# thiagopbueno/tf-mpc

Hardware: AMD Instinct MI355X
Metric: iLQR iterations/sec (batch x horizon) at n=16,m=8,T=50 (higher is better)
Workload: dtype f32

## Files before the change

### tf-mpc_amd/csrc/lqr_mfma16x8.hip

```cpp
#include <hip/hip_runtime.h>

#include <cstdlib>
#include <cstring>
#include <type_traits>

#include "lqr_kernels.h"
#include "options.h"
#include "mfma_bf16x3.h"
#include "wave_ldlt8.h"
#include "wave_ops.h"

namespace tfmpc {

namespace {

constexpr int N = 16, M = 8, D = 24;
using f32x4 = bf3::f32x4;

__device__ __forceinline__ f32x4 mfma(float a, float b, f32x4 c)
{
    return __builtin_amdgcn_mfma_f32_16x16x4f32(a, b, c, 0, 0, 0);
}

__device__ __forceinline__ float readlane(float v, int lane)
{
    return __builtin_bit_cast(float, __builtin_amdgcn_readlane(__builtin_bit_cast(int, v), lane));
}

using namespace bf3;

constexpr int kMs = 0;
constexpr int kKs = 256;
constexpr int kZs = 512;
constexpr int kZld = 26;
constexpr int kVtLd = 20;
#ifndef TFMPC_LQR_TC
#define TFMPC_LQR_TC 52
#endif
constexpr int kTC = TFMPC_LQR_TC;
constexpr int kLdsFloats = kZs + (kTC + 1) * kZld + 6;
#ifndef TFMPC_LQR_RING
#define TFMPC_LQR_RING 4
#endif
constexpr int kRing = TFMPC_LQR_RING;
static_assert(kTC % kRing == 0, "a chunk must hold whole turns of the gain ring");

template <int CTRL>
__device__ __forceinline__ float dpp(float v)
{
    return __builtin_bit_cast(float, __builtin_amdgcn_update_dpp(0, __builtin_bit_cast(int, v), CTRL, 0xF, 0xF, false));
}
constexpr int kDppXor1 = 0xB1;
constexpr int kDppXor2 = 0x4E;
constexpr int kDppHalfMirror = 0x141;

#define TFMPC_GLOBAL __attribute__((address_space(1)))
using gbytes = TFMPC_GLOBAL char *;
__device__ __forceinline__ gbytes uniform_base(const float *p)
{
    gbytes g = (gbytes)p;
    asm("" : "+s"(g));
    return g;
}
__device__ __forceinline__ unsigned here(unsigned &off)
{
    asm volatile("" : "+v"(off));
    return off;
}
template <class V>
__device__ __forceinline__ V gload(gbytes base, unsigned &off) { return *reinterpret_cast<const TFMPC_GLOBAL V *>(base + here(off)); }
template <class V>
__device__ __forceinline__ void gstore(gbytes base, unsigned &off, V v) { *reinterpret_cast<TFMPC_GLOBAL V *>(base + here(off)) = v; }
__device__ __forceinline__ int pinned(int v)
{
    asm("" : "+v"(v));
    return v;
}
typedef float f32x4_lds __attribute__((ext_vector_type(4), aligned(8)));
typedef float f32x4_any __attribute__((ext_vector_type(4), aligned(4)));

#ifdef TFMPC_LQR_EU
#define TFMPC_LQR_WAVES(EU_) TFMPC_LQR_EU
#else
#define TFMPC_LQR_WAVES(EU_) (EU_)
#endif
#define TFMPC_LQR_OCCUPANCY __attribute__((amdgpu_waves_per_eu(TFMPC_LQR_WAVES(EU), TFMPC_LQR_WAVES(EU))))
template <bool BACKWARD, bool FORWARD, bool VALUE, bool EXACT, bool BF3, bool OUT16 = false, int EU = 4>
__global__ __launch_bounds__(kWave) TFMPC_LQR_OCCUPANCY void lqr_mfma16x8_kernel(LqrArgs a)
{
    __shared__ __attribute__((aligned(16))) float lds[kLdsFloats];
    const int b = blockIdx.x;
    const int lane = threadIdx.x;
    const int i = lane & 15, q = lane >> 4;
    const int T = a.T;
    const int n = EXACT ? N : a.n, m = EXACT ? M : a.m, d = n + m;
    auto Fxx = [&](const float *Fg, int row, int xi) { return (row < n && xi < n) ? Fg[row * d + xi] : 0.0f; };
    auto Fxu = [&](const float *Fg, int row, int ui) { return (row < n && ui < m) ? Fg[row * d + n + ui] : 0.0f; };
    auto zmap = [&](int zi) { return zi < N ? (zi < n ? zi : -1) : (zi - N < m ? n + zi - N : -1); };
    auto Czz = [&](const float *Cg, int zr, int zc) {
        const int r = zmap(zr), c_ = zmap(zc);
        return (r >= 0 && c_ >= 0) ? Cg[r * d + c_] : 0.0f;
    };
    auto cz = [&](const float *cg, int zr) { const int r = zmap(zr); return r >= 0 ? cg[r] : 0.0f; };
    const float *Fg = a.F + (size_t)b * a.sF;
    const float *fg = a.f + (size_t)b * a.sf;
    const float *Cg = a.C + (size_t)b * a.sC;
    const float *cg = a.c + (size_t)b * a.sc;
    float *Kg = a.K + (size_t)b * a.sK;
    float *kg = a.k + (size_t)b * a.sk;
    int status = 0;

    if (BACKWARD) {
        float Fb0[4], Fb1[4];
        f32x4 Cd00, Cd11;
        f32x4 Cd01t;
        f32x4 vterm;
#pragma unroll
        for (int r = 0; r < 4; ++r) {
            const int k = 4 * q + r;
            const int ku = N + k;
            if (EXACT) {
                Fb0[r] = Fg[k * D + i];
                Fb1[r] = (i < M) ? Fg[k * D + N + i] : ((i == M) ? fg[k] : 0.0f);
                Cd00[r] = Cg[k * D + i];
                Cd01t[r] = (k < M) ? Cg[(N + k) * D + i] : ((k == M) ? cg[i] : 0.0f);
                vterm[r] = (i == M) ? cg[k] : 0.0f;
                Cd11[r] = (ku < D) ? ((i < M) ? Cg[ku * D + N + i] : ((i == M) ? cg[ku] : 0.0f)) : 0.0f;
            } else {
                Fb0[r] = Fxx(Fg, k, i);
                Fb1[r] = (i < M) ? Fxu(Fg, k, i) : ((i == M && k < n) ? fg[k] : 0.0f);
                Cd00[r] = Czz(Cg, k, i);
                Cd01t[r] = (k < M) ? Czz(Cg, N + k, i) : ((k == M) ? cz(cg, i) : 0.0f);
                vterm[r] = (i == M) ? cz(cg, k) : 0.0f;
                float c11 = 0.0f;
                if (ku < D) {
                    if (i < M) c11 = (k >= m && i == k) ? 1.0f : Czz(Cg, ku, N + i);
                    else if (i == M) c11 = cz(cg, ku);
                }
                Cd11[r] = c11;
            }
        }
        ConstFrag Fc0{}, Fc1{};
        if (BF3) {
            Fc0 = const_frag(f32x4{Fb0[0], Fb0[1], Fb0[2], Fb0[3]});
            Fc1 = const_frag(f32x4{Fb1[0], Fb1[1], Fb1[2], Fb1[3]});
        }
        f32x4 Vd = Cd00, vd = vterm;
        float cst = 0.0f;
        int min_pivot_bits = 0x3f800000;
        constexpr int kZero = kMs + 25 * 8;
        if (lane < kKs - kZero) lds[kZero + lane] = 0.0f;
        constexpr int kQx = kMs + 28 * 8;
        const int t01_src = (i == M) ? kQx + 4 * q : kZero;
        const int g1_src = (i == M) ? kKs + (N + M) * 8 + q : kZero + q;
        const int g0_src = pinned(kKs + i * 8 + q);
        const int vt_dst = pinned(kZs + 4 * q * kVtLd + i);
        unsigned offK = 8u * lane, offk = 4u * lane;
        __syncthreads();

        auto sweep_step = [&](const int t, auto LAST) __attribute__((always_inline)) {
            f32x4 W0 = {0.f, 0.f, 0.f, 0.f}, W1 = vd;
            if (BF3) {
                const VarFrag Vf = var_frag_block(Vd);
                W0 = mm_var_const(Vf, Fc0, W0);
                W1 = mm_var_const(Vf, Fc1, W1);
            } else {
#pragma unroll
                for (int r = 0; r < 4; ++r) {
                    W0 = mfma(Vd[r], Fb0[r], W0);
                    W1 = mfma(Vd[r], Fb1[r], W1);
                }
            }
            float fw = 0.0f, fv = 0.0f;
            if (VALUE) {
                float pw = 0.0f, pv = 0.0f;
#pragma unroll
                for (int r = 0; r < 4; ++r) {
                    pw = fmaf(Fb1[r], W1[r], pw);
                    pv = fmaf(Fb1[r], vd[r], pv);
                }
                fw = wave_sum(i == M ? pw : 0.0f);
                fv = wave_sum(i == M ? pv : 0.0f);
            }
            f32x4 T00 = Cd00, T01t = Cd01t, T11 = Cd11;
            if (BF3) {
                const VarFrag W0f = var_frag_block(W0), W1f = var_frag_block(W1);
                T00 = mm_const_var(Fc0, W0f, T00);
                T01t = mm_var_const(W1f, Fc0, T01t);
                T11 = mm_const_var(Fc1, W1f, T11);
            } else {
#pragma unroll
                for (int r = 0; r < 4; ++r) {
                    T00 = mfma(Fb0[r], W0[r], T00);
                    T01t = mfma(W1[r], Fb0[r], T01t);
                    T11 = mfma(Fb1[r], W1[r], T11);
                }
            }
            if (q < 2) {
                *reinterpret_cast<f32x4 *>(&lds[kMs + i * 8 + 4 * q]) = T01t;
                if (i <= M) *reinterpret_cast<f32x4 *>(&lds[kMs + (N + i) * 8 + 4 * q]) = T11;
            } else if (q == 2) {
                lds[kQx + i] = T01t[0];
            }
            lds_sync();
            f32x2 M2[4];
            {
                const int c = lane & 31;
                const f32x4 lo = *reinterpret_cast<const f32x4 *>(&lds[kMs + c * 8]);
                const f32x4 hi = *reinterpret_cast<const f32x4 *>(&lds[kMs + c * 8 + 4]);
                M2[0] = f32x2{lo[0], lo[1]}; M2[1] = f32x2{lo[2], lo[3]};
                M2[2] = f32x2{hi[0], hi[1]}; M2[3] = f32x2{hi[2], hi[3]};
            }
            float quk = 0.0f;
            float qu_saved[8];
            if (VALUE) {
#pragma unroll
                for (int p = 0; p < 8; ++p) qu_saved[p] = readlane(M2[p >> 1][p & 1], 24);
            }
            float Mr[8];
            ldlt8_solve_neg(M2, Mr, min_pivot_bits);
            if (VALUE) {
#pragma unroll
                for (int p = 0; p < 8; ++p) quk = fmaf(readlane(Mr[p], 24), qu_saved[p], quk);
            }
            if (lane < 32) {
                f32x4 lo, hi;
#pragma unroll
                for (int r = 0; r < 4; ++r) { lo[r] = Mr[r]; hi[r] = Mr[4 + r]; }
                *reinterpret_cast<f32x4 *>(&lds[kKs + lane * 8]) = lo;
                *reinterpret_cast<f32x4 *>(&lds[kKs + lane * 8 + 4]) = hi;
            }
            lds_sync();
            if constexpr (!decltype(LAST)::value) {
                f32x4 vacc = *reinterpret_cast<const f32x4 *>(&lds[t01_src]);
#pragma unroll
                for (int s2 = 0; s2 < 2; ++s2) {
                    const float ax = lds[kMs + i * 8 + 4 * s2 + q];
                    const float g0 = lds[g0_src + 4 * s2];
                    const float g1 = lds[g1_src + 4 * s2];
                    T00 = mfma(ax, g0, T00);
                    vacc = mfma(ax, g1, vacc);
                }
                {
                    const float *vt = &lds[kZs];
#pragma unroll
                    for (int r = 0; r < 4; ++r) lds[vt_dst + r * kVtLd] = T00[r];
                    lds_sync();
                    const f32x4 Tt = *reinterpret_cast<const f32x4 *>(&vt[i * kVtLd + 4 * q]);
#pragma unroll
                    for (int r = 0; r < 4; ++r) Vd[r] = 0.5f * (T00[r] + Tt[r]);
                }
                vd = vacc;
            }
            {
                const int ka = lane >> 3, jc = lane & 7;
                float2 kv;
                kv.x = lds[kKs + (2 * jc) * 8 + ka];
                kv.y = lds[kKs + (2 * jc + 1) * 8 + ka];
                if (EXACT) {
                    gstore(uniform_base(Kg + (size_t)t * (M * N)), offK, f32x2{kv.x, kv.y});
                    if (lane < M) gstore(uniform_base(kg + (size_t)t * M), offk, lds[kKs + 24 * 8 + lane]);
                } else {
                    if (ka < m && 2 * jc < n) Kg[(size_t)t * m * n + ka * n + 2 * jc] = kv.x;
                    if (ka < m && 2 * jc + 1 < n) Kg[(size_t)t * m * n + ka * n + 2 * jc + 1] = kv.y;
                    if (lane < m) kg[(size_t)t * m + lane] = lds[kKs + 24 * 8 + lane];
                }
                if (OUT16 && a.K16) {
                    uint16_t *Ko = a.K16 + ((size_t)b * T + t) * (m * n);
                    if (ka < m && 2 * jc < n) Ko[ka * n + 2 * jc] = lqr_to_bf16(kv.x);
                    if (ka < m && 2 * jc + 1 < n) Ko[ka * n + 2 * jc + 1] = lqr_to_bf16(kv.y);
                }
                if (OUT16 && a.k16 && lane < m) a.k16[((size_t)b * T + t) * m + lane] = lqr_to_bf16(lds[kKs + 24 * 8 + lane]);
            }
            if (VALUE) {
                cst += 0.5f * quk + 0.5f * (fw + fv);
                if (a.V) {
                    float *Vo = a.V + ((size_t)b * T + t) * (n * n);
#pragma unroll
                    for (int r = 0; r < 4; ++r)
                        if (EXACT || (4 * q + r < n && i < n)) Vo[(4 * q + r) * n + i] = Vd[r];
                }
                if (a.v && i == M) {
                    float *vo = a.v + ((size_t)b * T + t) * n;
#pragma unroll
                    for (int r = 0; r < 4; ++r)
                        if (EXACT || 4 * q + r < n) vo[4 * q + r] = vd[r];
                }
                if (a.cst && lane == 0) a.cst[(size_t)b * T + t] = cst;
                if (OUT16 && a.V16) {
                    uint16_t *Vo = a.V16 + ((size_t)b * T + t) * (n * n);
#pragma unroll
                    for (int r = 0; r < 4; ++r)
                        if (EXACT || (4 * q + r < n && i < n)) Vo[(4 * q + r) * n + i] = lqr_to_bf16(Vd[r]);
                }
                if (OUT16 && a.v16 && i == M) {
                    uint16_t *vo = a.v16 + ((size_t)b * T + t) * n;
#pragma unroll
                    for (int r = 0; r < 4; ++r)
                        if (EXACT || 4 * q + r < n) vo[4 * q + r] = lqr_to_bf16(vd[r]);
                }
                if (OUT16 && a.cst16 && lane == 0) a.cst16[(size_t)b * T + t] = lqr_to_bf16(cst);
            }
            lds_sync();
        };
        constexpr int kPeeled = VALUE ? 0 : 1;
        for (int t = T - 1; t >= kPeeled; --t) sweep_step(t, std::false_type{});
        if (kPeeled && T > 0) sweep_step(0, std::true_type{});
        if (min_pivot_bits <= 0) status |= (min_pivot_bits == 0) ? TFMPC_ST_SINGULAR : TFMPC_ST_NOT_PD;
        if (VALUE && !(cst == cst)) status |= TFMPC_ST_NAN;
    }

    if (FORWARD) {
        const int fi = lane >> 2, fc = lane & 3;
        const int ka = lane >> 3, jc = lane & 7;
        float Fr[6];
        if (EXACT) {
            const float2 *p = reinterpret_cast<const float2 *>(Fg + fi * D + 6 * fc);
#pragma unroll
            for (int j = 0; j < 3; ++j) { const float2 v = p[j]; Fr[2 * j] = v.x; Fr[2 * j + 1] = v.y; }
        } else {
#pragma unroll
            for (int j = 0; j < 6; ++j) {
                const int zc = 6 * fc + j;
                Fr[j] = zc < N ? Fxx(Fg, fi, zc) : Fxu(Fg, fi, zc - N);
            }
        }
        const float f_part = (fc == 0 && (EXACT || fi < n)) ? fg[fi] : 0.0f;
        float Ca0[6], Ca1[6];
        f32x4 cq0, cq1;
#pragma unroll
        for (int s2 = 0; s2 < 6; ++s2) {
            if (EXACT) {
                Ca0[s2] = Cg[i * D + 4 * s2 + q];
                Ca1[s2] = (i < M) ? Cg[(N + i) * D + 4 * s2 + q] : 0.0f;
            } else {
                Ca0[s2] = Czz(Cg, i, 4 * s2 + q);
                Ca1[s2] = (i < M) ? Czz(Cg, N + i, 4 * s2 + q) : 0.0f;
            }
        }
#pragma unroll
        for (int r = 0; r < 4; ++r) {
            cq0[r] = EXACT ? cg[4 * q + r] : cz(cg, 4 * q + r);
            cq1[r] = (q < 2) ? (EXACT ? cg[N + 4 * q + r] : cz(cg, N + 4 * q + r)) : 0.0f;
        }
        float *xs = a.states + (size_t)b * (T + 1) * n;
        float *us = a.actions + (size_t)b * T * m;
        float *cs = a.costs + (size_t)b * (T + 1);
        float *zs = &lds[kZs];
        __syncthreads();
        if (lane < N) {
            const float x = (EXACT || lane < n) ? a.x0[(size_t)b * n + lane] : 0.0f;
            zs[lane] = x;
            if (EXACT || lane < n) xs[lane] = x;
        }
        unsigned offK = 8u * lane, offk = 4u * ka;
        auto load_gain = [&](int t, float2 &Kv, float &kv) {
            if (EXACT) {
                const f32x2 K2 = gload<f32x2>(uniform_base(Kg + (size_t)t * (M * N)), offK);
                Kv = float2{K2[0], K2[1]};
                kv = gload<float>(uniform_base(kg + (size_t)t * M), offk);
            } else {
                const bool row = ka < m;
                Kv.x = (row && 2 * jc < n) ? Kg[(size_t)t * m * n + ka * n + 2 * jc] : 0.0f;
                Kv.y = (row && 2 * jc + 1 < n) ? Kg[(size_t)t * m * n + ka * n + 2 * jc + 1] : 0.0f;
                kv = row ? kg[(size_t)t * m + ka] : 0.0f;
            }
        };
        float2 KR[kRing];
        float kR[kRing];
#pragma unroll
        for (int d = 0; d < kRing; ++d) {
            KR[d] = float2{0.f, 0.f};
            kR[d] = 0.0f;
            if (T > 0) load_gain(d < T ? d : T - 1, KR[d], kR[d]);
        }
        __syncthreads();

        auto chunk_costs = [&](int rows, float *out) {
            for (int nt = 0; nt * 16 < rows; ++nt) {
                const int row = (16 * nt + i < rows) ? 16 * nt + i : rows - 1;
                const float *zrow = zs + row * kZld;
                f32x4 D0 = {0.f, 0.f, 0.f, 0.f}, D1 = {0.f, 0.f, 0.f, 0.f};
#pragma unroll
                for (int s2 = 0; s2 < 6; ++s2) {
                    const float bz = zrow[4 * s2 + q];
                    D0 = mfma(Ca0[s2], bz, D0);
                    D1 = mfma(Ca1[s2], bz, D1);
                }
                float part = 0.0f;
#pragma unroll
                for (int r = 0; r < 4; ++r) {
                    part = fmaf(zrow[4 * q + r], fmaf(0.5f, D0[r], cq0[r]), part);
                    if (q < 2) part = fmaf(zrow[N + 4 * q + r], fmaf(0.5f, D1[r], cq1[r]), part);
                }
                part += __shfl_xor(part, 16, kWave);
                part += __shfl_xor(part, 32, kWave);
                if (q == 0 && 16 * nt + i < rows) out[16 * nt + i] = part;
            }
        };

        auto rollout_step = [&](const int tt, const int t, float2 &KRd, float &kRd, auto REFILL) __attribute__((always_inline)) {
            float *zt = zs + tt * kZld;
            const float2 Kc = KRd;
            const float kc = kRd;
            const float2 xv = *reinterpret_cast<const float2 *>(&zt[2 * jc]);
            float u = fmaf(Kc.x, xv.x, Kc.y * xv.y);
            u += dpp<kDppXor1>(u);
            u += dpp<kDppXor2>(u);
            u += dpp<kDppHalfMirror>(u);
            u += kc;
            if constexpr (decltype(REFILL)::value) load_gain(t + kRing < T ? t + kRing : T - 1, KRd, kRd);
            zt[N + ka] = u;
            lds_sync();
            float xn = f_part;
            const float2 *zp = reinterpret_cast<const float2 *>(&zt[6 * fc]);
#pragma unroll
            for (int j = 0; j < 3; ++j) {
                const float2 z2 = zp[j];
                xn = fmaf(Fr[2 * j], z2.x, xn);
                xn = fmaf(Fr[2 * j + 1], z2.y, xn);
            }
            xn += dpp<kDppXor1>(xn);
            xn += dpp<kDppXor2>(xn);
            zt[kZld + fi] = xn;
            lds_sync();
        };

        const int xrow = lane >> 2, urow = lane >> 1;
        const float *xsrc = zs + (1 + xrow) * kZld + 4 * (lane & 3);
        const float *usrc = zs + urow * kZld + N + 4 * (lane & 1);
        unsigned off16 = 16u * lane;

        for (int t0 = 0; t0 < T; t0 += kTC) {
            const int tc = (T - t0 < kTC) ? (T - t0) : kTC;
            int tb = 0;
            for (; tb + kRing <= tc; tb += kRing) {
#pragma unroll
                for (int d = 0; d < kRing; ++d) rollout_step(tb + d, t0 + tb + d, KR[d], kR[d], std::true_type{});
            }
#pragma unroll
            for (int d = 0; d < kRing - 1; ++d)
                if (tb + d < tc) rollout_step(tb + d, t0 + tb + d, KR[d], kR[d], std::false_type{});
            chunk_costs(tc, cs + t0);
            if (EXACT) {
                const gbytes xdst = uniform_base(xs + (size_t)(t0 + 1) * N), udst = uniform_base(us + (size_t)t0 * M);
#pragma unroll
                for (int r0 = 0; r0 < kTC; r0 += kWave / 4) {
                    if (r0 >= tc) break;
                    if (r0 + xrow < tc)
                        gstore<f32x4_any>(xdst + r0 * (N * 4), off16, *reinterpret_cast<const f32x4_lds *>(xsrc + r0 * kZld));
                }
#pragma unroll
                for (int r0 = 0; r0 < kTC; r0 += kWave / 2) {
                    if (r0 >= tc) break;
                    if (r0 + urow < tc)
                        gstore<f32x4_any>(udst + r0 * (M * 4), off16, *reinterpret_cast<const f32x4_lds *>(usrc + r0 * kZld));
                }
            } else {
                for (int idx = lane; idx < tc * n; idx += kWave)
                    xs[(size_t)(t0 + 1) * n + idx] = zs[(1 + idx / n) * kZld + idx % n];
                for (int idx = lane; idx < tc * m; idx += kWave)
                    us[(size_t)t0 * m + idx] = zs[(idx / m) * kZld + N + idx % m];
            }
            lds_sync();
            if (lane < N) zs[lane] = zs[tc * kZld + lane];
            lds_sync();
        }
        if (lane < M) zs[N + lane] = 0.0f;
        lds_sync();
        chunk_costs(1, cs + T);
        lds_sync();
        if (lane == 0) {
            const float fcost = cs[T];
            if (!(fcost == fcost)) status |= TFMPC_ST_NAN;
        }
    }

    if (a.status && lane == 0) a.status[b] = status;
}

bool use_bf16x3()
{
    return !option_is(kOptLqrMfma, "f32");
}

int pick_eu()
{
    const int forced = option_int(kOptLqrWaves, 0);
    return forced == 4 ? 4 : 5;
}

template <bool BW, bool FW, bool VAL, bool O16, int EU>
int launch_eu(const LqrArgs &a, hipStream_t stream)
{
    const bool exact = a.n == N && a.m == M;
    const bool bf3 = BW && use_bf16x3();
    const dim3 grid(a.B), block(kWave);
    if (exact && bf3) hipLaunchKernelGGL((lqr_mfma16x8_kernel<BW, FW, VAL, true, true, O16, EU>), grid, block, 0, stream, a);
    else if (exact) hipLaunchKernelGGL((lqr_mfma16x8_kernel<BW, FW, VAL, true, false, O16, EU>), grid, block, 0, stream, a);
    else if (bf3) hipLaunchKernelGGL((lqr_mfma16x8_kernel<BW, FW, VAL, false, true, O16, EU>), grid, block, 0, stream, a);
    else hipLaunchKernelGGL((lqr_mfma16x8_kernel<BW, FW, VAL, false, false, O16, EU>), grid, block, 0, stream, a);
    return hipGetLastError() == hipSuccess ? TFMPC_OK : TFMPC_ERR_LAUNCH;
}

template <bool BW, bool FW, bool VAL, bool O16 = false>
int launch(const LqrArgs &a, hipStream_t stream)
{
    if constexpr (!VAL) {
        if (pick_eu() == 5) return launch_eu<BW, FW, VAL, O16, 5>(a, stream);
    }
    return launch_eu<BW, FW, VAL, O16, 4>(a, stream);
}

}

bool lqr_mfma_supported(int n, int m) { return n >= 1 && m >= 1 && n <= N && m <= M && n + m > 6; }

int lqr_mfma_launch(const LqrArgs &a, bool backward, bool forward, hipStream_t stream)
{
    if (a.K16 || a.k16 || a.V16 || a.v16 || a.cst16) {
        if (backward && forward) return launch<true, true, true, true>(a, stream);
        if (backward) return launch<true, false, true, true>(a, stream);
    }
    const bool value = a.V || a.v || a.cst;
    if (backward && forward) return value ? launch<true, true, true>(a, stream) : launch<true, true, false>(a, stream);
    if (backward) return value ? launch<true, false, true>(a, stream) : launch<true, false, false>(a, stream);
    return launch<false, true, false>(a, stream);
}

}
```

Baseline: 39.95 million.

## Pair two batch elements per workgroup and alternate LDLT solve between waves

Launches two waves per workgroup, each handling its own batch element in the backward sweep without value outputs. The 8x8 LDLT elimination is replaced by a paired variant in which one wave, alternating by time step, solves both elements' systems using DPP row broadcasts, one element per 32-lane half. Block barriers synchronize the two waves around the solve, and pivot minima are merged at the end. This targets the poorly utilized serial solve on the critical path, at the cost of workgroup-wide barriers, doubled LDS per block and a dead wave when B is odd.

```diff
diff --git a/tf-mpc_amd/csrc/lqr_mfma16x8.hip b/tf-mpc_amd/csrc/lqr_mfma16x8.hip
--- a/tf-mpc_amd/csrc/lqr_mfma16x8.hip
+++ b/tf-mpc_amd/csrc/lqr_mfma16x8.hip
@@ -8,6 +8,7 @@
 #include "options.h"
 #include "mfma_bf16x3.h"
 #include "wave_ldlt8.h"
+#include "wave_ldlt8_pair.h"
 #include "wave_ops.h"
 
 namespace tfmpc {
@@ -85,12 +86,23 @@
 #define TFMPC_LQR_WAVES(EU_) (EU_)
 #endif
 #define TFMPC_LQR_OCCUPANCY __attribute__((amdgpu_waves_per_eu(TFMPC_LQR_WAVES(EU), TFMPC_LQR_WAVES(EU))))
-template <bool BACKWARD, bool FORWARD, bool VALUE, bool EXACT, bool BF3, bool OUT16 = false, int EU = 4>
-__global__ __launch_bounds__(kWave) TFMPC_LQR_OCCUPANCY void lqr_mfma16x8_kernel(LqrArgs a)
-{
-    __shared__ __attribute__((aligned(16))) float lds[kLdsFloats];
-    const int b = blockIdx.x;
-    const int lane = threadIdx.x;
+__device__ __forceinline__ void block_lds_sync()
+{
+    __builtin_amdgcn_fence(__ATOMIC_RELEASE, "workgroup", "local");
+    __builtin_amdgcn_s_barrier();
+    __builtin_amdgcn_fence(__ATOMIC_ACQUIRE, "workgroup", "local");
+}
+template <bool BACKWARD, bool FORWARD, bool VALUE, bool EXACT, bool BF3, bool OUT16 = false, int EU = 4, bool PAIR = false>
+__global__ __launch_bounds__(PAIR ? 2 * kWave : kWave) TFMPC_LQR_OCCUPANCY void lqr_mfma16x8_kernel(LqrArgs a)
+{
+    static_assert(!PAIR || (BACKWARD && !VALUE && !OUT16), "the paired elimination serves the sweeps without value outputs");
+    __shared__ __attribute__((aligned(16))) float lds_all[(PAIR ? 2 : 1) * kLdsFloats];
+    const int wave = PAIR ? __builtin_amdgcn_readfirstlane(threadIdx.x >> 6) : 0;
+    float *const lds = lds_all + wave * kLdsFloats;
+    const int b_own = PAIR ? 2 * (int)blockIdx.x + wave : (int)blockIdx.x;
+    const bool live = !PAIR || b_own < a.B;
+    const int b = live ? b_own : a.B - 1;
+    const int lane = PAIR ? (int)(threadIdx.x & (kWave - 1)) : (int)threadIdx.x;
     const int i = lane & 15, q = lane >> 4;
     const int T = a.T;
     const int n = EXACT ? N : a.n, m = EXACT ? M : a.m, d = n + m;
@@ -148,6 +160,11 @@
         f32x4 Vd = Cd00, vd = vterm;
         float cst = 0.0f;
         int min_pivot_bits = 0x3f800000;
+        int min_pivot_rows = 0x3f800000;
+        const int pj = lane & 15, prow = (lane >> 4) & 1;
+        const int pcol = pj >= 8 ? pj - 8 + 8 * prow : ((prow && pj == 0) ? N + M : N + pj);
+        const int pair_src = PAIR ? 4 * pinned(((lane >> 5) * kLdsFloats + kMs + pcol * 8) / 4) : 0;
+        const int pair_d0 = (lane >> 5) * kLdsFloats + kMs + N * 8;
         constexpr int kZero = kMs + 25 * 8;
         if (lane < kKs - kZero) lds[kZero + lane] = 0.0f;
         constexpr int kQx = kMs + 28 * 8;
@@ -202,35 +219,55 @@
             } else if (q == 2) {
                 lds[kQx + i] = T01t[0];
             }
-            lds_sync();
-            f32x2 M2[4];
-            {
-                const int c = lane & 31;
-                const f32x4 lo = *reinterpret_cast<const f32x4 *>(&lds[kMs + c * 8]);
-                const f32x4 hi = *reinterpret_cast<const f32x4 *>(&lds[kMs + c * 8 + 4]);
-                M2[0] = f32x2{lo[0], lo[1]}; M2[1] = f32x2{lo[2], lo[3]};
-                M2[2] = f32x2{hi[0], hi[1]}; M2[3] = f32x2{hi[2], hi[3]};
-            }
             float quk = 0.0f;
-            float qu_saved[8];
-            if (VALUE) {
-#pragma unroll
-                for (int p = 0; p < 8; ++p) qu_saved[p] = readlane(M2[p >> 1][p & 1], 24);
-            }
-            float Mr[8];
-            ldlt8_solve_neg(M2, Mr, min_pivot_bits);
-            if (VALUE) {
-#pragma unroll
-                for (int p = 0; p < 8; ++p) quk = fmaf(readlane(Mr[p], 24), qu_saved[p], quk);
-            }
-            if (lane < 32) {
-                f32x4 lo, hi;
-#pragma unroll
-                for (int r = 0; r < 4; ++r) { lo[r] = Mr[r]; hi[r] = Mr[4 + r]; }
-                *reinterpret_cast<f32x4 *>(&lds[kKs + lane * 8]) = lo;
-                *reinterpret_cast<f32x4 *>(&lds[kKs + lane * 8 + 4]) = hi;
-            }
-            lds_sync();
+            if constexpr (PAIR) {
+                block_lds_sync();
+                if (wave == (t & 1)) {
+                    f32x2 P2[4];
+                    const f32x4 lo = *reinterpret_cast<const f32x4 *>(&lds_all[pair_src]);
+                    const f32x4 hi = *reinterpret_cast<const f32x4 *>(&lds_all[pair_src + 4]);
+                    const float d0 = lds_all[pair_d0];
+                    P2[0] = f32x2{lo[0], lo[1]}; P2[1] = f32x2{lo[2], lo[3]};
+                    P2[2] = f32x2{hi[0], hi[1]}; P2[3] = f32x2{hi[2], hi[3]};
+                    float Pr[8];
+                    ldlt8_pair_solve_neg(P2, Pr, d0, min_pivot_rows);
+                    f32x4 klo, khi;
+#pragma unroll
+                    for (int r = 0; r < 4; ++r) { klo[r] = Pr[r]; khi[r] = Pr[4 + r]; }
+                    *reinterpret_cast<f32x4 *>(&lds_all[pair_src + (kKs - kMs)]) = klo;
+                    *reinterpret_cast<f32x4 *>(&lds_all[pair_src + (kKs - kMs) + 4]) = khi;
+                }
+                block_lds_sync();
+            } else {
+                lds_sync();
+                f32x2 M2[4];
+                {
+                    const int c = lane & 31;
+                    const f32x4 lo = *reinterpret_cast<const f32x4 *>(&lds[kMs + c * 8]);
+                    const f32x4 hi = *reinterpret_cast<const f32x4 *>(&lds[kMs + c * 8 + 4]);
+                    M2[0] = f32x2{lo[0], lo[1]}; M2[1] = f32x2{lo[2], lo[3]};
+                    M2[2] = f32x2{hi[0], hi[1]}; M2[3] = f32x2{hi[2], hi[3]};
+                }
+                float qu_saved[8];
+                if (VALUE) {
+#pragma unroll
+                    for (int p = 0; p < 8; ++p) qu_saved[p] = readlane(M2[p >> 1][p & 1], 24);
+                }
+                float Mr[8];
+                ldlt8_solve_neg(M2, Mr, min_pivot_bits);
+                if (VALUE) {
+#pragma unroll
+                    for (int p = 0; p < 8; ++p) quk = fmaf(readlane(Mr[p], 24), qu_saved[p], quk);
+                }
+                if (lane < 32) {
+                    f32x4 lo, hi;
+#pragma unroll
+                    for (int r = 0; r < 4; ++r) { lo[r] = Mr[r]; hi[r] = Mr[4 + r]; }
+                    *reinterpret_cast<f32x4 *>(&lds[kKs + lane * 8]) = lo;
+                    *reinterpret_cast<f32x4 *>(&lds[kKs + lane * 8 + 4]) = hi;
+                }
+                lds_sync();
+            }
             if constexpr (!decltype(LAST)::value) {
                 f32x4 vacc = *reinterpret_cast<const f32x4 *>(&lds[t01_src]);
 #pragma unroll
@@ -252,7 +289,7 @@
                 }
                 vd = vacc;
             }
-            {
+            if (live) {
                 const int ka = lane >> 3, jc = lane & 7;
                 float2 kv;
                 kv.x = lds[kKs + (2 * jc) * 8 + ka];
@@ -306,6 +343,13 @@
         constexpr int kPeeled = VALUE ? 0 : 1;
         for (int t = T - 1; t >= kPeeled; --t) sweep_step(t, std::false_type{});
         if (kPeeled && T > 0) sweep_step(0, std::true_type{});
+        if constexpr (PAIR) {
+            constexpr int kMinPv = kKs + 25 * 8;
+            if ((lane & 31) == 0) lds[kMinPv + (lane >> 5)] = __builtin_bit_cast(float, min_pivot_rows);
+            block_lds_sync();
+            const int p0 = __builtin_bit_cast(int, lds_all[kMinPv + wave]), p1 = __builtin_bit_cast(int, lds_all[kLdsFloats + kMinPv + wave]);
+            min_pivot_bits = __builtin_amdgcn_readfirstlane(p0 < p1 ? p0 : p1);
+        }
         if (min_pivot_bits <= 0) status |= (min_pivot_bits == 0) ? TFMPC_ST_SINGULAR : TFMPC_ST_NOT_PD;
         if (VALUE && !(cst == cst)) status |= TFMPC_ST_NAN;
     }
@@ -351,7 +395,7 @@
         if (lane < N) {
             const float x = (EXACT || lane < n) ? a.x0[(size_t)b * n + lane] : 0.0f;
             zs[lane] = x;
-            if (EXACT || lane < n) xs[lane] = x;
+            if (live && (EXACT || lane < n)) xs[lane] = x;
         }
         unsigned offK = 8u * lane, offk = 4u * ka;
         auto load_gain = [&](int t, float2 &Kv, float &kv) {
@@ -395,7 +439,7 @@
                 }
                 part += __shfl_xor(part, 16, kWave);
                 part += __shfl_xor(part, 32, kWave);
-                if (q == 0 && 16 * nt + i < rows) out[16 * nt + i] = part;
+                if (live && q == 0 && 16 * nt + i < rows) out[16 * nt + i] = part;
             }
         };
 
@@ -442,7 +486,8 @@
             for (int d = 0; d < kRing - 1; ++d)
                 if (tb + d < tc) rollout_step(tb + d, t0 + tb + d, KR[d], kR[d], std::false_type{});
             chunk_costs(tc, cs + t0);
-            if (EXACT) {
+            if (!live) {
+            } else if (EXACT) {
                 const gbytes xdst = uniform_base(xs + (size_t)(t0 + 1) * N), udst = uniform_base(us + (size_t)t0 * M);
 #pragma unroll
                 for (int r0 = 0; r0 < kTC; r0 += kWave / 4) {
@@ -470,13 +515,13 @@
         lds_sync();
         chunk_costs(1, cs + T);
         lds_sync();
-        if (lane == 0) {
+        if (live && lane == 0) {
             const float fcost = cs[T];
             if (!(fcost == fcost)) status |= TFMPC_ST_NAN;
         }
     }
 
-    if (a.status && lane == 0) a.status[b] = status;
+    if (live && a.status && lane == 0) a.status[b] = status;
 }
 
 bool use_bf16x3()
@@ -495,11 +540,12 @@
 {
     const bool exact = a.n == N && a.m == M;
     const bool bf3 = BW && use_bf16x3();
-    const dim3 grid(a.B), block(kWave);
-    if (exact && bf3) hipLaunchKernelGGL((lqr_mfma16x8_kernel<BW, FW, VAL, true, true, O16, EU>), grid, block, 0, stream, a);
-    else if (exact) hipLaunchKernelGGL((lqr_mfma16x8_kernel<BW, FW, VAL, true, false, O16, EU>), grid, block, 0, stream, a);
-    else if (bf3) hipLaunchKernelGGL((lqr_mfma16x8_kernel<BW, FW, VAL, false, true, O16, EU>), grid, block, 0, stream, a);
-    else hipLaunchKernelGGL((lqr_mfma16x8_kernel<BW, FW, VAL, false, false, O16, EU>), grid, block, 0, stream, a);
+    constexpr bool P = BW && !VAL && !O16;
+    const dim3 grid(P ? (a.B + 1) / 2 : a.B), block(P ? 2 * kWave : kWave);
+    if (exact && bf3) hipLaunchKernelGGL((lqr_mfma16x8_kernel<BW, FW, VAL, true, true, O16, EU, P>), grid, block, 0, stream, a);
+    else if (exact) hipLaunchKernelGGL((lqr_mfma16x8_kernel<BW, FW, VAL, true, false, O16, EU, P>), grid, block, 0, stream, a);
+    else if (bf3) hipLaunchKernelGGL((lqr_mfma16x8_kernel<BW, FW, VAL, false, true, O16, EU, P>), grid, block, 0, stream, a);
+    else hipLaunchKernelGGL((lqr_mfma16x8_kernel<BW, FW, VAL, false, false, O16, EU, P>), grid, block, 0, stream, a);
     return hipGetLastError() == hipSuccess ? TFMPC_OK : TFMPC_ERR_LAUNCH;
 }
 
diff --git a/tf-mpc_amd/csrc/wave_ldlt8_pair.h b/tf-mpc_amd/csrc/wave_ldlt8_pair.h
--- /dev/null
+++ b/tf-mpc_amd/csrc/wave_ldlt8_pair.h
@@ -0,0 +1,75 @@
+#pragma once
+
+#include <hip/hip_runtime.h>
+
+#include <utility>
+
+#include "wave_ldlt8.h"
+
+namespace tfmpc {
+
+template <int L>
+__device__ __forceinline__ float rcp_neg_row_bcast(float v)
+{
+    static_assert(L >= 0 && L < 16, "a row has 16 lanes");
+    float r;
+    asm("s_nop 1\n\tv_rcp_f32_dpp %0, -%1 row_newbcast:%2 row_mask:0xf bank_mask:0xf\n\ts_nop 0" : "=v"(r) : "v"(v), "n"(L));
+    return r;
+}
+template <int L>
+__device__ __forceinline__ int min_row_bcast(int v, int m)
+{
+    static_assert(L >= 0 && L < 16, "a row has 16 lanes");
+    asm("s_nop 1\n\tv_min_i32_dpp %0, %1, %0 row_newbcast:%2 row_mask:0xf bank_mask:0xf" : "+v"(m) : "v"(v), "n"(L));
+    return m;
+}
+template <int L>
+__device__ __forceinline__ float fma_row_bcast(float v, float b, float acc)
+{
+    static_assert(L >= 0 && L < 16, "a row has 16 lanes");
+    asm("s_nop 1\n\tv_fmac_f32_dpp %0, %1, %2 row_newbcast:%3 row_mask:0xf bank_mask:0xf" : "+v"(acc) : "v"(v), "v"(b), "n"(L));
+    return acc;
+}
+
+namespace ldlt8_pair_detail {
+template <class F, int... I>
+__device__ __forceinline__ void static_for(F &&f, std::integer_sequence<int, I...>) { (f(std::integral_constant<int, I>{}), ...); }
+}
+
+__device__ __forceinline__ void ldlt8_pair_solve_neg(f32x2 (&M2)[4], float (&X)[8], float d0, int &min_pivot_bits)
+{
+    using namespace ldlt8_pair_detail;
+    f32x2 N2[4];
+    static_for([&](auto P) {
+        constexpr int p = decltype(P)::value;
+        constexpr int pp = p >> 1, ps = p & 1;
+        const float Mp = M2[pp][ps];
+        float ninv;
+        if constexpr (p == 0) {
+            const int pvb = __builtin_bit_cast(int, d0);
+            min_pivot_bits = pvb < min_pivot_bits ? pvb : min_pivot_bits;
+            ninv = __builtin_amdgcn_rcpf(-d0);
+        } else {
+            min_pivot_bits = min_row_bcast<p>(__builtin_bit_cast(int, Mp), min_pivot_bits);
+            ninv = rcp_neg_row_bcast<p>(Mp);
+        }
+        const float Mn = Mp * ninv;
+        N2[pp][ps] = Mn;
+        static_for([&](auto S) {
+            constexpr int s = p + 1 + decltype(S)::value;
+            M2[s >> 1][s & 1] = fma_row_bcast<s>(Mn, Mp, M2[s >> 1][s & 1]);
+        }, std::make_integer_sequence<int, 7 - p>{});
+    }, std::make_integer_sequence<int, 8>{});
+    static_for([&](auto PP) {
+        constexpr int p = 6 - decltype(PP)::value;
+        const float O = N2[p >> 1][p & 1];
+        static_for([&](auto S) {
+            constexpr int s = 7 - decltype(S)::value;
+            N2[p >> 1][p & 1] = fma_row_bcast<s>(O, N2[s >> 1][s & 1], N2[p >> 1][p & 1]);
+        }, std::make_integer_sequence<int, 7 - p>{});
+    }, std::make_integer_sequence<int, 7>{});
+#pragma unroll
+    for (int r = 0; r < 8; ++r) X[r] = N2[r >> 1][r & 1];
+}
+
+}
```

Result: faster. 42.01 million (median of 6 runs) (+5.2%).
